# darrelllong/Delta-Compression

Measured on AMD Instinct MI355X. Metric: delta-encode GiB/s (device-resident batched pairs) at 1/2/4/8 MI355X, higher is better.
Workload: dtype u8; 1 GPU; 4096 x 64 KiB pairs per GPU, 1% edits, onepass, --table-size 1; algorithm=onepass, pairs_per_gpu=4096, pairs_total=4096, pair_bytes=65536, q=4099, parallelism=dp1 (pair shards, RCCL index scatter + size all-gather)

## Files before the change

### delta-compression_amd/__init__.py

```python
from __future__ import annotations

from ._lib import (
    ALGO_CORRECTING,
    ALGO_GREEDY,
    ALGO_ONEPASS,
    BUF_CAP,
    MAX_TABLE_SIZE,
    SEED_LEN,
    TABLE_SIZE,
    AddCmd,
    Context,
    CopyCmd,
    PlacedAdd,
    PlacedCopy,
    DeltaError,
    DiffOptions,
    EncodePlan,
    DecodePlan,
    InplacePlan,
    UpdatePlan,
    ComposeDesc,
    ComposePlan,
    InvertDesc,
    InvertPlan,
    SplicePlan,
    ReadPlan,
    ReadReq,
    ReadStream,
    SketchPlan,
    SKETCH_BINS,
    SKETCH_EMPTY,
    MATCH_NONE,
    MATCH_ALL,
    MATCH_NOT_SELF,
    MATCH_EARLIER,
    LIB_PATH,
    LIMIT_ONEPASS_MEMBERS,
    LIMIT_TABLE_POOL_BYTES,
    MEMBERS_AUTO,
    MEMBERS_OFF,
    MEMBERS_ON,
    crc64_xz,
    decode,
    decode_delta,
    default_context,
    diff,
    diff_correcting,
    diff_greedy,
    diff_onepass,
    diff_placed,
    encode,
# ... 35 lines not shown
    unplace_commands,
)

__all__ = [
    "ALGO_ONEPASS", "ALGO_CORRECTING", "ALGO_GREEDY", "SEED_LEN", "TABLE_SIZE",
    "MAX_TABLE_SIZE", "BUF_CAP", "Context", "DeltaError", "DiffOptions", "EncodePlan", "DecodePlan", "InplacePlan", "UpdatePlan",
    "ComposeDesc", "ComposePlan", "compose", "compose_batch",
    "InvertDesc", "InvertPlan", "invert", "invert_batch",
    "SplicePlan", "segment_pairs", "splice", "splice_batch", "sketch_windows", "encode_large",
    "ReadPlan", "ReadReq", "ReadStream", "read_range", "read_ranges", "tile_requests", "decode_large",
    "LineagePlan", "read_lineage", "read_lineage_batch", "lineage_work_items", "LINEAGE_BASE", "LINEAGE_MAX_DEPTH",
    "SketchPlan", "sketch", "sketch_batch", "match_sketches", "match_sketches_device", "pick_bases", "SKETCH_BINS", "SKETCH_EMPTY",
    "MATCH_NONE", "MATCH_ALL", "MATCH_NOT_SELF", "MATCH_EARLIER",
    "crc64_xz", "decode", "default_context", "encode", "encode_batch", "encode_pipelined", "info", "lib",
    "make_inplace", "make_inplace_batch", "update_batch", "status_string", "LIB_PATH", "LIMIT_TABLE_POOL_BYTES",
    "LIMIT_ONEPASS_MEMBERS", "MEMBERS_AUTO", "MEMBERS_ON", "MEMBERS_OFF",
    "CopyCmd", "AddCmd", "PlacedCopy", "PlacedAdd", "diff", "diff_greedy", "diff_onepass", "diff_correcting",
    "diff_placed", "place_commands", "unplace_commands", "output_size", "encode_delta", "decode_delta",
]
```

### delta-compression_amd/_lib.py

```python
from __future__ import annotations

import ctypes as C
import os
import threading
from dataclasses import dataclass
from typing import Iterable, List, Optional, Sequence, Tuple

HERE = os.path.dirname(os.path.abspath(__file__))
_VARIANT = os.environ.get("DG_LIB_VARIANT", "")
LIB_PATH = os.path.join(HERE, "lib", "libdeltagpu%s.so" % ("_" + _VARIANT if _VARIANT else ""))

ALGO_GREEDY, ALGO_ONEPASS, ALGO_CORRECTING = 0, 1, 2
SEED_LEN = 16
TABLE_SIZE = 1048573
MAX_TABLE_SIZE = 1073741827
BUF_CAP = 256
OPT_VERBOSE, OPT_SPLAY, OPT_INPLACE, OPT_POLICY_CONSTANT = 0, 1, 2, 3
POLICIES = {"localmin": 0, "constant": 1}
CMD_COPY, CMD_ADD = 0, 1
SKETCH_BINS = 256
SKETCH_EMPTY = 0xFFFFFFFFFFFFFFFF
MATCH_NONE = 0xFFFFFFFF
MATCH_ALL, MATCH_NOT_SELF, MATCH_EARLIER = 0, 1, 2
_MATCH_MODES = {"all": MATCH_ALL, "not_self": MATCH_NOT_SELF, "earlier": MATCH_EARLIER}

_ALGOS = {"greedy": ALGO_GREEDY, "onepass": ALGO_ONEPASS, "correcting": ALGO_CORRECTING}

STATUS = {
    0: "DG_OK", 1: "DG_ERR_INVALID_ARG", 2: "DG_ERR_UNSUPPORTED", 3: "DG_ERR_TOO_LARGE",
    4: "DG_ERR_NO_DEVICE", 5: "DG_ERR_HIP", 6: "DG_ERR_NOMEM", 7: "DG_ERR_CAPACITY",
    8: "DG_ERR_MALFORMED", 9: "DG_ERR_SRC_CRC", 10: "DG_ERR_DST_CRC", 11: "DG_ERR_TABLE_POOL", 12: "DG_ERR_INTERNAL",
}
LIMIT_TABLE_POOL_BYTES = 0
LIMIT_ONEPASS_MEMBERS = 1
MEMBERS_AUTO, MEMBERS_ON, MEMBERS_OFF = 0, 1, 2


class DeltaError(RuntimeError):
    def __init__(self, code: int, msg: str = ""):
        self.code = code
        super().__init__(f"{STATUS.get(code, code)}: {msg}" if msg else STATUS.get(code, str(code)))


class DiffOptions(C.Structure):
    _fields_ = [("p", C.c_size_t), ("q", C.c_size_t), ("buf_cap", C.c_size_t),
                ("max_table", C.c_size_t), ("flags", C.c_uint64)]

    @classmethod
    def make(cls, p: int = SEED_LEN, q: int = TABLE_SIZE, buf_cap: int = BUF_CAP,
# ... 1378 lines not shown
```

### delta-compression_amd/csrc/dg_crc.h

```cpp
#pragma once
#include <hip/hip_runtime.h>
#include <stdint.h>

#include <type_traits>

#include "dg_device.h"
#include "dg_devutil.h"

namespace dg {

typedef const __attribute__((address_space(3))) uint64_t lds_cu64;
__device__ __forceinline__ uint64_t ldsq(uint32_t a) { return *(lds_cu64*)(size_t)a; }
__device__ __forceinline__ uint32_t lds_addr(const void* p) {
	return (uint32_t)(size_t)(lds_cu64*)(const uint64_t*)p;
}

__device__ __forceinline__ uint64_t byte_mask(int lo, int hi) {
	lo = lo < 0 ? 0 : lo;
	hi = hi > 8 ? 8 : hi;
	if (hi <= lo) return 0;
	const uint64_t up = hi == 8 ? ~0ULL : ((1ULL << (8 * hi)) - 1);
	const uint64_t dn = lo == 0 ? 0ULL : ((1ULL << (8 * lo)) - 1);
	return up & ~dn;
}
// ... 55 lines not shown
		five(v, ylo, yhi, tb);
		if constexpr (PB == 16) five(v + 13, h0, h1, tb + 13 * 256);
	}
	uint32_t l[N + 1], h[N + 1];
#pragma unroll
	for (int k = 0; k < N; ++k) {
		l[k] = (uint32_t)v[k];
		h[k] = (uint32_t)(v[k] >> 32);
	}
	l[N] = xlo;
	h[N] = xhi;
	ylo = xor_tree<N + 1>(l);
	yhi = xor_tree<N + 1>(h);
}

template <uint32_t PB, uint32_t NC, int kPf, uint32_t SEG = kCrcSegBytes, bool kCopy = false, int TAB = kCrcByte>
__device__ __forceinline__ uint64_t crc_seg_rows(uintptr_t start, uint64_t len, uint32_t nseg, uint32_t j,
                                                 uint32_t tb, uint32_t tbh, uint64_t klane,
                                                 intptr_t copy_delta = 0, uintptr_t copy_hi = 0) {
	static_assert(PB == 8 || PB == 16, "piece bytes");
	static_assert(!kCopy || PB == 8, "copy: 8-byte pieces");
	static_assert(TAB == kCrcByte || NC == 1, "five-bit tables: one copy");
	constexpr uint32_t RB = 64 * PB, NR = SEG / RB;
	static_assert(NR % (2 * kPf) == 0, "two batches of rows per loop");
	const uint32_t lane = lane_id();
	const uintptr_t end = start + len;
	const uintptr_t a0 = start & ~(uintptr_t)15;
	const uintptr_t a1 = (end + 15) & ~(uintptr_t)15;
	const uintptr_t dom = a1 - (uintptr_t)nseg * SEG;
	const uintptr_t p0 = dom + (uintptr_t)j * SEG + (uintptr_t)lane * PB;
	auto clamp32 = [](intptr_t v) -> int32_t {
		return (int32_t)(v < -(intptr_t)RB ? -(intptr_t)RB : (v > (intptr_t)(SEG + RB) ? (intptr_t)(SEG + RB) : v));
	};
	const int32_t f0 = clamp32((intptr_t)start - (intptr_t)p0);
	const int32_t l0 = clamp32((intptr_t)end - (intptr_t)p0);
	const int32_t z0 = clamp32((intptr_t)a0 - (intptr_t)p0);
	typedef uint32_t v4u __attribute__((ext_vector_type(4)));
	typedef uint32_t v2u __attribute__((ext_vector_type(2)));
	typedef typename std::conditional<PB == 16, v4u, v2u>::type piece_t;
	typedef __attribute__((address_space(1))) const piece_t gpiece;
	uint32_t ylo = 0, yhi = 0, h0 = 0, h1 = 0;
	auto fold_piece = [&](const piece_t& p, uint32_t inv) {
		if constexpr (PB == 16) {
			crc_fold<TAB, PB, NC>(ylo, yhi, h0, h1, p.x ^ inv, p.y ^ inv, tb, tbh);
			h0 = p.z;
			h1 = p.w;
		} else {
			crc_fold<TAB, PB, NC>(ylo, yhi, h0, h1, p.x ^ inv, p.y ^ inv, tb, tbh);
		}
	};
	auto copy = [&](const piece_t* xs, uint32_t r0) {
		if constexpr (kCopy) {
#pragma unroll
			for (int u = 0; u < kPf; ++u) {
				const uintptr_t pa = p0 + (uintptr_t)(r0 + u) * RB;
				if (pa >= start && pa + PB <= copy_hi)
					*reinterpret_cast<__attribute__((address_space(1))) v2u*>(pa + copy_delta) = xs[u];
			}
		}
	};
	const bool edge = (j == 0 && dom != start) || (j + 1 == nseg && end != a1);
	if (!edge) {
		const uint32_t inv = j == 0 && lane == 0 ? ~0u : 0u;
		piece_t xa[kPf], xb[kPf];
		auto load = [&](piece_t* xs, uint32_t r0) {
#pragma unroll
			for (int u = 0; u < kPf; ++u) xs[u] = *reinterpret_cast<gpiece*>(p0 + (uintptr_t)(r0 + u) * RB);
		};
		auto consume = [&](const piece_t* xs, uint32_t r0) {
			copy(xs, r0);
			fold_piece(xs[0], r0 == 0 ? inv : 0u);
#pragma unroll
			for (int u = 1; u < kPf; ++u) fold_piece(xs[u], 0u);
		};
		load(xa, 0);
		for (uint32_t r0 = 0; r0 < NR; r0 += 2 * kPf) {
			load(xb, r0 + kPf);
			consume(xa, r0);
			if (r0 + 2 * kPf < NR) load(xa, r0 + 2 * kPf);
			consume(xb, r0 + kPf);
		}
	} else {
		for (uint32_t r0 = 0; r0 < NR; r0 += kPf) {
			piece_t xs[kPf];
#pragma unroll
			for (int u = 0; u < kPf; ++u) {
				const int32_t o = (int32_t)((r0 + u) * RB);
				xs[u] = piece_t{};
// ... 12 lines not shown
					const int lc = max(min(l, 24), -8);
					uint64_t lo = ((uint64_t)x.y << 32) | x.x, hi = ((uint64_t)x.w << 32) | x.z;
					lo &= byte_mask(fc, lc);
					hi &= byte_mask(fc - 8, lc - 8);
					lo ^= byte_mask(fc, fc + 8);
					hi ^= byte_mask(fc - 8, fc);
					x = v4u{(uint32_t)lo, (uint32_t)(lo >> 32), (uint32_t)hi, (uint32_t)(hi >> 32)};
				}
				piece_t px;
				if constexpr (PB == 16) px = x;
				else px = piece_t{x.x, x.y};
				fold_piece(px, 0u);
			}
		}
	}
	crc_fold<TAB, PB, NC>(ylo, yhi, h0, h1, 0u, 0u, tb, tbh);
	const uint64_t A = ((uint64_t)yhi << 32) | ylo;
	return wave_xor64(A ? gf2_mulmod(A, klane) : 0ull);
}

}
```

### delta-compression_amd/csrc/dg_device.h

```cpp
#pragma once
#include <stdint.h>

#include "../../include/delta_gpu.h"
#include "dg_layout.h"

namespace dg {


struct EncodeArgs {
	const uint8_t* ref;
	const uint8_t* ver;
	const PairDev* pairs;
	const PairPlanDev* pplan;
	uint32_t n_pairs;
	uint32_t pair0;
	uint32_t p;
	const uint64_t* powc;
	uint32_t* rec;
	uint32_t* n_rec;
	uint64_t* dsize;
	int32_t* status;
	unsigned long long* tables;
	uint64_t qmax;
	uint32_t n_tables;
// ... 90 lines not shown
	uint32_t n_pairs;
};

struct CrcArgs {
	const uint8_t* arena[2];
	const CrcSpanDev* spans;
	const CrcSegDev* segs;
	uint32_t n_segs;
	uint32_t n_spans;
	const uint64_t* tables;
	uint64_t* seg_crc;
	uint64_t* out;
	const uint64_t* xinv;
	uint64_t kseg;
	const uint32_t* prio_flag;
};

struct dg_decode_desc_dev {
	uint64_t ref_off, ref_len;
	uint64_t delta_off, delta_len;
	uint64_t out_off, out_cap;
};

struct DecodeArgs {
	const uint8_t* ref;
	const uint8_t* delta;
	const dg_decode_desc_dev* descs;
	uint32_t n;
	uint8_t* out;
	uint64_t* out_len;
// ... 17 lines not shown

hipError_t launch_onepass(const EncodeArgs& a, uint32_t p, bool aligned16, hipStream_t st,
                          hipEvent_t routed_after = nullptr);
bool onepass16_selected();
hipError_t launch_members(const SpecArgs& a, uint32_t n_chunks, uint32_t n_cu, hipStream_t st);
hipError_t launch_member_serialize(const MemSerArgs& a, uint32_t n_chunks, uint32_t n_cu, hipStream_t st);
hipError_t launch_correcting_clear(const EncodeArgs& a, hipStream_t st);
hipError_t launch_correcting(const EncodeArgs& a, uint32_t p, hipStream_t st, uint32_t lds_cap, uint64_t qmin,
                             hipEvent_t ev_built, hipEvent_t ev_fork);
hipError_t launch_greedy(const GreedyArgs& g, uint64_t head_words, hipStream_t st, hipEvent_t ev_built);
hipError_t launch_scan(const uint64_t* sz, uint64_t* off, uint32_t n, hipStream_t st,
                       uint32_t* route_cnt = nullptr, uint32_t* route_fb = nullptr);
hipError_t launch_serialize_wave(const SerArgs& s, hipStream_t st);
hipError_t launch_crc_patch(uint8_t* out, const uint64_t* offsets, const uint64_t* crc,
                            const int32_t* status, uint32_t n, hipStream_t st);
enum : int { kCrcPassRows = 0, kCrcPassRows5 = 1 };
hipError_t launch_crc(const CrcArgs& a, hipStream_t st, uint32_t overlap_cap = 0, int pass = kCrcPassRows,
                      bool finalize = true);
hipError_t launch_crc_finalize(const CrcArgs& a, hipStream_t st);
hipError_t launch_crc_wide(const CrcArgs& a, uint32_t n_cu, hipStream_t st);
hipError_t launch_decode(const DecodeArgs& a, hipStream_t st);
hipError_t launch_synth(uint8_t* ref, uint8_t* ver, uint32_t n_pairs, uint64_t pair_len,
                        uint64_t seed_base, uint64_t n_edits, hipStream_t st);
hipError_t launch_synth_shift(uint8_t* ref, uint8_t* ver, const SynthSpan* spans, const uint64_t* v_off,
                              uint32_t n, uint64_t n_edits, uint32_t pct, hipStream_t st);
hipError_t launch_synth_transpose(uint8_t* ref, uint8_t* ver, const SynthSpan* spans, uint32_t n_spans,
                                  const SynthCopy* cmds, uint32_t n_cmds, hipStream_t st);

}
```

### delta-compression_amd/csrc/dg_host.cpp

```cpp
#include <dlfcn.h>
#include <hip/hip_runtime.h>

#include <algorithm>
#include <cstdarg>
#include <cstdio>
#include <cstdlib>
#include <new>
#include <string>
#include <vector>

#include "../../include/delta_gpu.h"
#include "dg_device.h"
#include "dg_hostutil.h"
#include "dg_plan.h"

using namespace dg;


struct dg_context {
	int device = -1;
	hipStream_t stream = nullptr;
	uint64_t* d_crc_tables = nullptr;
	uint64_t* d_xinv = nullptr;
	uint64_t* d_k32 = nullptr;
	uint64_t kseg = 0;
	uint32_t n_cu = 256;
	int lds_bytes = 0;
	uint64_t table_pool_bytes = 0;
	uint64_t onepass_members = 0;
	uint64_t limits_gen = 0;
	std::string err;
	void* pin = nullptr;
	size_t pin_cap = 0;
	void* io = nullptr;
	void (*io_free)(void*) = nullptr;
	void* module[kCtxModules] = {};
	void (*module_free[kCtxModules])(void*) = {};
};

uint64_t dg::ctx_limits_gen(const dg_context_t* ctx) { return ctx->limits_gen; }
int dg::ctx_device(const dg_context_t* ctx) { return ctx->device; }

void** dg::ctx_io(dg_context_t* ctx, void (*release)(void*)) {
	ctx->io_free = release;
// ... 117 lines not shown
	delete ctx;
}

void* dg_context_stream(dg_context_t* ctx) { return ctx ? (void*)ctx->stream : nullptr; }

int dg_context_set_limit(dg_context_t* ctx, int limit, uint64_t value) {
	if (!ctx) return DG_ERR_INVALID_ARG;
	switch (limit) {
	case DG_LIMIT_TABLE_POOL_BYTES:
		ctx->table_pool_bytes = value;
		++ctx->limits_gen;
		return DG_OK;
	case DG_LIMIT_ONEPASS_MEMBERS:
		if (value > 2) return set_err(ctx, DG_ERR_INVALID_ARG, "onepass members mode %llu", (unsigned long long)value);
		ctx->onepass_members = value;
		++ctx->limits_gen;
		return DG_OK;
	default: return set_err(ctx, DG_ERR_INVALID_ARG, "unknown limit %d", limit);
	}
}

}

const char* dg::ab_env(const char* name) {
#ifdef DG_AB_SWITCHES
	return getenv(name);
#else
	(void)name;
	return nullptr;
#endif
// ... 71 lines not shown
		return 0;
	}
	uint32_t read() const { return __atomic_load_n(h, __ATOMIC_RELAXED); }
};

}


struct dg_encode_plan {
	dg_context_t* ctx = nullptr;
	dg_algorithm_t algo = DG_ALGO_ONEPASS;
	dg_diff_options_t opts{};
	uint32_t n = 0;
	EncodeGeometry g;
	std::vector<dg_pair_t> pairs;
	DevBuf d_pairs, d_pplan, d_powc, d_rec, d_nrec, d_dsize, d_crc_spans_r, d_crc_segs,
	    d_seg_crc, d_crc, d_tables, d_locks, d_tags, d_ctab, d_lookback, d_kcls, d_gpairs, d_prio_flag,
	    d_gent;
	DevBuf d_mem_s, d_srec, d_nmem, d_chunks, d_csum, d_cmap, d_seg, d_nseg;
	hipStream_t side = nullptr;
	hipEvent_t ev_fork = nullptr, ev_join = nullptr;
	bool serial_crc = false;
	bool skip_crc = false;
	DevBuf d_route_cnt;
	HostWord route_fb;
	uint32_t plain_streak = 0;
	uint64_t member_runs = 0, plain_runs = 0;
	uint64_t* stats = nullptr;
	int timing_mode = DG_TIMING_ALL;
	TimingRing ring;
// ... 15 lines not shown
#ifndef DG_CRC_PRIO_FLAG
#define DG_CRC_PRIO_FLAG 0
#endif
constexpr bool kCrcPrioFlag = DG_CRC_PRIO_FLAG != 0;

static int plan_fill(dg_encode_plan_t* P, const dg_pair_t* pairs) {
	dg_context_t* ctx = P->ctx;
	const dg_algorithm_t algo = P->algo;
	const uint32_t n = P->n;
	EncodeGeometry& g = P->g;
	PlanEnv env;
	env.n_cu = ctx->n_cu;
	env.lds_bytes = ctx->lds_bytes;
	env.table_pool_bytes = ctx->table_pool_bytes;
	env.onepass_members = ctx->onepass_members;
	env.onepass16 = onepass16_selected();
	env.no_members = ab_env("DG_NO_MEMBERS");
	env.members = ab_env("DG_MEMBERS");
	env.corr_build = ab_env("DG_CORR_BUILD");
	env.fused = ab_env("DG_FUSED");
	env.route_min = ab_env("DG_ROUTE_MIN");
	std::string err;
	const int rc = encode_geometry(algo, P->opts, pairs, n, env, g, err);
	if (rc != DG_OK) {
		if (!err.empty()) ctx->err = err;
		return rc;
	}
	hipSetDevice(ctx->device);

	const uint32_t n1 = std::max<uint32_t>(n, 1);
	const size_t p = P->opts.p;
	int bad = 0;
	bad |= P->d_pairs.alloc(sizeof(PairDev) * n1);
	bad |= P->d_pplan.alloc(sizeof(PairPlanDev) * n1);
	bad |= P->d_powc.alloc(8 * p);
	bad |= P->d_rec.alloc(4ull * (algo != DG_ALGO_CORRECTING ? kRecWordsOnepass : kRecWordsCorrecting) *
	                      std::max<uint64_t>(g.total_rec, 1));
	bad |= P->d_nrec.alloc(4ull * n1);
	bad |= P->d_dsize.alloc(8ull * n1);
	bad |= P->d_crc_spans_r.alloc(sizeof(CrcSpanDev) * std::max<size_t>(g.spans.size(), 1));
	bad |= P->d_crc_segs.alloc(sizeof(CrcSegDev) * std::max<size_t>(g.segs.size(), 1));
	bad |= P->d_seg_crc.alloc(8 * std::max<size_t>(g.segs.size(), 1));
	bad |= P->d_crc.alloc(16ull * n1);
	bad |= P->d_tables.alloc(g.table_bytes * g.n_tables);
	bad |= P->d_locks.alloc(4ull * g.n_tables);
	bad |= P->d_tags.alloc(4ull * g.n_tables);
	if (algo == DG_ALGO_CORRECTING) {
		bad |= P->d_gpairs.alloc(4ull * std::max<size_t>(g.gpairs.size(), 1));
		if (!bad && !g.gpairs.empty() &&
		    hipMemcpy(P->d_gpairs.p, g.gpairs.data(), 4 * g.gpairs.size(), hipMemcpyHostToDevice) != hipSuccess)
			bad = 1;
		bad |= P->d_ctab.alloc(4ull * std::max<uint64_t>(g.ctab_entries, 1));
		bad |= P->d_kcls.alloc(8ull * n1);
	}
	if (g.fused) bad |= P->d_lookback.alloc(8ull * n1);
	if (algo == DG_ALGO_GREEDY) {
		bad |= P->d_ctab.alloc(4ull * std::max<uint64_t>(g.greedy_heads, 1));
// ... 28 lines not shown
			g.members = false;
			g.n_chunks = 0;
			mbad = 0;
		}
		bad |= mbad;
	}
	if (bad) return set_err(ctx, DG_ERR_NOMEM, "device allocation failed");
	hipStream_t st = ctx->stream;
	hipError_t e = hipSuccess;
	if (n) {
		e = hipMemcpyAsync(P->d_pairs.p, pairs, sizeof(PairDev) * n, hipMemcpyHostToDevice, st);
		if (e == hipSuccess) e = hipMemcpyAsync(P->d_pplan.p, g.pp.data(), sizeof(PairPlanDev) * n, hipMemcpyHostToDevice, st);
		if (e == hipSuccess) e = hipMemcpyAsync(P->d_crc_spans_r.p, g.spans.data(), sizeof(CrcSpanDev) * g.spans.size(), hipMemcpyHostToDevice, st);
		if (e == hipSuccess && !g.segs.empty()) e = hipMemcpyAsync(P->d_crc_segs.p, g.segs.data(), sizeof(CrcSegDev) * g.segs.size(), hipMemcpyHostToDevice, st);
	}
	if (e == hipSuccess) e = hipMemcpyAsync(P->d_powc.p, g.powc.data(), 8 * p, hipMemcpyHostToDevice, st);
	if (e == hipSuccess) e = hipMemsetAsync(P->d_tables.p, 0, P->d_tables.n, st);
	if (e == hipSuccess) e = hipMemsetAsync(P->d_locks.p, 0, P->d_locks.n, st);
	if (e == hipSuccess) e = hipMemsetAsync(P->d_tags.p, 0, P->d_tags.n, st);
	if (e == hipSuccess) e = hipStreamSynchronize(st);
	if (e != hipSuccess) return set_err(ctx, DG_ERR_HIP, "plan upload failed: %s", hipGetErrorString(e));
	const char* sc = ab_env("DG_SERIAL_CRC");
	P->serial_crc = sc && sc[0] == '1';
	const char* sk = ab_env("DG_SKIP_CRC");
	P->skip_crc = sk && sk[0] == '1';

	if (!P->serial_crc) {
		e = hipStreamCreateWithFlags(&P->side, hipStreamNonBlocking);
		if (e == hipSuccess) e = hipEventCreateWithFlags(&P->ev_fork, hipEventDisableTiming | hipEventReleaseToDevice);
		if (e == hipSuccess) e = hipEventCreateWithFlags(&P->ev_join, hipEventDisableTiming | hipEventReleaseToDevice);
// ... 243 lines not shown
	const bool chain_join = mem && !serial && !P->skip_crc && P->g.route_min && P->route_fb.read() > 16u * ctx->n_cu;

	CrcArgs c{};
	c.arena[0] = d_ref;
	c.arena[1] = d_ver;
	c.spans = P->d_crc_spans_r.as<CrcSpanDev>();
	c.segs = P->d_crc_segs.as<CrcSegDev>();
	c.n_segs = (uint32_t)P->g.segs.size();
	c.n_spans = (uint32_t)P->g.spans.size();
	c.tables = ctx->d_crc_tables;
	c.seg_crc = P->d_seg_crc.as<uint64_t>();
	c.out = P->d_crc.as<uint64_t>();
	c.xinv = ctx->d_xinv;
	c.kseg = ctx->kseg;
	c.prio_flag = kCrcPrioFlag && mem ? P->d_prio_flag.as<uint32_t>() : nullptr;
	auto run_crc = [&]() -> int {
		HIPCHK(ctx, rec(0, cs));
		if (!P->skip_crc) {
			const uint32_t rounds = (P->n + 16u * ctx->n_cu - 1) / (16u * ctx->n_cu);
			const uint32_t cap = serial || P->g.crc_fused ? 0u : 2u * ctx->n_cu * std::max(rounds, 1u);
			HIPCHK(ctx, launch_crc(c, cs, cap, mem ? kCrcPassRows5 : kCrcPassRows, !late_fin));
		}
		HIPCHK(ctx, rec(1, cs));
		if (!serial) HIPCHK(ctx, hipEventRecord(P->ev_join, cs));
		return DG_OK;
	};
	auto run_diff = [&]() -> int {
		HIPCHK(ctx, rec(2, st));
		if (!mem) HIPCHK(ctx, rec(6, st));
		EncodeArgs a{};
		a.ref = d_ref;
		a.ver = d_ver;
		a.pairs = P->d_pairs.as<PairDev>();
		a.pplan = P->d_pplan.as<PairPlanDev>();
		a.n_pairs = P->n;
		a.p = (uint32_t)P->opts.p;
// ... 276 lines not shown
```

### delta-compression_amd/csrc/dg_kernels.hip

```cpp
#include <hip/hip_runtime.h>
#include <stdint.h>

#include <type_traits>

#include "dg_device.h"
#include "dg_devutil.h"
#include "dg_crc.h"
#include "dg_serialize_wave.h"

namespace dg {


__device__ __forceinline__ uint64_t wave_incl_scan64(uint64_t x) {
	const uint32_t lane = lane_id();
#pragma unroll
	for (int d = 1; d < 64; d <<= 1) {
		const uint32_t lo = (uint32_t)__shfl_up((int)(uint32_t)x, d, 64);
		const uint32_t hi = (uint32_t)__shfl_up((int)(uint32_t)(x >> 32), d, 64);
		if (lane >= (uint32_t)d) x += ((uint64_t)hi << 32) | lo;
	}
	return x;
}

__global__ __launch_bounds__(1024) void scan_sizes_kernel(const uint64_t* __restrict__ sz,
// ... 73 lines not shown
	for (uint32_t seg = uni(blockIdx.x * kCrcWavesPerBlock + wave); seg < a.n_segs;
	     seg += gridDim.x * kCrcWavesPerBlock) {
		if (a.prio_flag && !raised) {
			if (uni(__hip_atomic_load(a.prio_flag, __ATOMIC_RELAXED, __HIP_MEMORY_SCOPE_AGENT))) {
				__builtin_amdgcn_s_setprio(1);
				raised = true;
			}
		}
		const CrcSegDev sd = a.segs[seg];
		const CrcSpanDev sp = a.spans[sd.span];
		const uint64_t c = crc_seg_rows<8, 1, TAB == kCrcByte ? DG_CRC_PF : DG_CRC_PF5, kCrcSegBytes, false, TAB>(
		    (uintptr_t)(a.arena[sp.which] + sp.off), sp.len, sp.nseg, sd.j, tb, tb, kl);
		if (lane == 0) a.seg_crc[seg] = c;
	}
}

__global__ __launch_bounds__(64) void crc_finalize_kernel(CrcArgs a) {
	const uint32_t i = blockIdx.x * 64 + threadIdx.x;
	if (i >= a.n_spans) return;
	const CrcSpanDev sp = a.spans[i];
	uint64_t crc;
	if (sp.len < 8) {
		const uint8_t* d = a.arena[sp.which] + sp.off;
		uint64_t c = ~0ULL;
		for (uint64_t k = 0; k < sp.len; ++k) c = a.tables[(uint8_t)(c ^ d[k])] ^ (c >> 8);
		crc = ~c;
	} else {
		const uint64_t* KS = a.tables + 8 * 256 + kCrcLevels * kCrcNibTabWords;
		uint64_t acc = 0;
		for (uint32_t j = 0; j < sp.nseg; ++j)
// ... 223 lines not shown

hipError_t launch_crc_finalize(const CrcArgs& a, hipStream_t st) {
	if (a.n_spans) hipLaunchKernelGGL(crc_finalize_kernel, dim3((a.n_spans + 63) / 64), dim3(64), 0, st, a);
	return hipGetLastError();
}

hipError_t launch_crc(const CrcArgs& a, hipStream_t st, uint32_t overlap_cap, int pass, bool finalize) {
	if (a.n_segs) {
		uint32_t blocks = (a.n_segs + kCrcWavesPerBlock - 1) / kCrcWavesPerBlock;
		static const uint32_t env_cap = [] {
			const char* e = ab_env("DG_CRC_BLOCKS");
			return e ? (uint32_t)strtoul(e, nullptr, 0) : 0u;
		}();
		const uint32_t cap = env_cap ? env_cap : overlap_cap;
		if (cap && blocks > cap) blocks = cap;
		if (pass == kCrcPassRows5)
			hipLaunchKernelGGL(crc_rows_kernel<kCrcFive>, dim3(blocks), dim3(64 * kCrcWavesPerBlock), 0, st, a);
		else
			hipLaunchKernelGGL(crc_rows_kernel<kCrcByte>, dim3(blocks), dim3(64 * kCrcWavesPerBlock), 0, st, a);
	}
	if (finalize) return launch_crc_finalize(a, st);
	return hipGetLastError();
}

hipError_t launch_synth(uint8_t* ref, uint8_t* ver, uint32_t n_pairs, uint64_t pair_len,
                        uint64_t seed_base, uint64_t n_edits, hipStream_t st) {
	const uint64_t words = (uint64_t)n_pairs * ((pair_len + 7) / 8);
	if (words)
		hipLaunchKernelGGL(synth_random_kernel, dim3((unsigned)((words + 255) / 256)), dim3(256), 0, st,
		                   ref, ver, pair_len, seed_base, words);
// ... 233 lines not shown
```

### delta-compression_amd/csrc/dg_layout.h

```cpp
#pragma once
#include <stdint.h>

namespace dg {

constexpr uint64_t kMersenne = (1ULL << 61) - 1;
constexpr uint64_t kBase = 263;
constexpr uint64_t kCrcPoly = 0xC96C5795D7870F42ULL;
constexpr uint32_t kSentinel = 0xFFFFFFFFu;

constexpr uint32_t kCrcSegBytes = 65536;
constexpr uint32_t kCrcWavesPerBlock = 4;

#ifndef DG_HIST_CHUNKS
#define DG_HIST_CHUNKS 6
#endif
constexpr int kHistChunks = DG_HIST_CHUNKS;

struct PairDev {
	uint64_t r_off, r_len, v_off, v_len;
};

struct PairPlanDev {
	uint64_t q;
	uint64_t q_magic;
// ... 2 lines not shown
	uint32_t pad;
	uint64_t f_size, f_magic;
	uint64_t m, m_magic;
	uint64_t tab_base;
	uint64_t mem_base;
	uint32_t chunk_base;
	uint32_t n_chunks;
	uint64_t crc_unpad;
};

struct CrcSegDev {
	uint32_t span;
	uint32_t j;
};

struct CrcSpanDev {
	uint64_t off, len;
	uint32_t seg_base;
	uint32_t nseg;
	uint32_t which;
	uint32_t out;
};

constexpr int kCrcLevels = 6;
constexpr int kCrcNibTabWords = 256;
constexpr int kCrcFinTabs = 1 + 16 + 3 + 3;
constexpr int kCrcFinX256 = 20, kCrcFinX512 = 21, kCrcFinX48K = 22;
constexpr uint32_t kCrcRowsOff = 8 * 256 + (kCrcLevels + kCrcFinTabs) * kCrcNibTabWords;
constexpr uint32_t kCrcRows16 = kCrcRowsOff, kCrcRows8 = kCrcRowsOff + 16 * 256;
constexpr uint32_t kCrcRowK16 = kCrcRowsOff + 24 * 256, kCrcRowK8 = kCrcRowK16 + 64;
// ... 22 lines not shown
```

### delta-compression_amd/csrc/dg_plan.cpp

```cpp
#include "dg_plan.h"

#include <algorithm>
#include <cstdarg>
#include <cstdio>
#include <cstdlib>
#include <cstring>
#include <map>

namespace dg {


namespace {

typedef unsigned __int128 u128;

uint64_t mulmod64(uint64_t a, uint64_t b, uint64_t m) { return (uint64_t)((u128)a * b % m); }

uint64_t powmod64(uint64_t b, uint64_t e, uint64_t m) {
	uint64_t r = 1 % m;
	b %= m;
	for (; e; e >>= 1) {
		if (e & 1) r = mulmod64(r, b, m);
		b = mulmod64(b, b, m);
	}
// ... 157 lines not shown
	seg.clear();
	for (size_t i = 0; i < spans.size(); ++i) {
		CrcSpanDev& s = sd[i];
		s.off = spans[i].off;
		s.len = spans[i].len;
		s.seg_base = (uint32_t)seg.size();
		s.nseg = 0;
		s.which = which[i];
		s.out = outs ? (*outs)[i] : (uint32_t)i;
		if (s.len >= 8) {
			const uint64_t a0 = s.off & ~15ull, a1 = (s.off + s.len + 15) & ~15ull;
			s.nseg = (uint32_t)((a1 - a0 + kCrcSegBytes - 1) / kCrcSegBytes);
			for (uint32_t j = 0; j < s.nseg; ++j) seg.push_back(CrcSegDev{(uint32_t)i, j});
		}
	}
}


namespace {

bool is_one(const char* v) { return v && v[0] == '1'; }

bool members_wanted(const PlanEnv& env, const dg_pair_t* pairs, uint32_t n) {
	uint64_t vsum = 0;
	for (uint32_t i = 0; i < n; ++i) vsum += pairs[i].v_len;
	bool want = n && vsum / n >= (128u << 10);
	if (env.onepass_members == 1) want = true;
	if (env.onepass_members == 2) want = false;
	if (is_one(env.no_members)) want = false;
	if (is_one(env.members)) want = true;
// ... 147 lines not shown
	if (g.members) {
		for (uint32_t i = 0; i < n; ++i) {
			const uint64_t E = std::min<uint64_t>(pairs[i].r_len, pairs[i].v_len);
			const uint32_t nch = (uint32_t)(E / kMemChunk + 1);
			g.pp[i].mem_base = g.mem_slots;
			g.pp[i].chunk_base = g.n_chunks;
			g.pp[i].n_chunks = nch;
			for (uint32_t c = 0; c < nch; ++c) {
				g.jobs.push_back(i);
				g.jobs.push_back(c);
			}
			g.mem_slots += (uint64_t)nch * kMemChunkSlots;
			g.n_chunks += nch;
		}
	}
	return DG_OK;
}


namespace {
void print_command_stats(const dg_commands_t& cmds) {
	uint64_t tc = 0, ta = 0, nc = 0, na = 0;
	std::vector<uint64_t> lens;
	for (size_t i = 0; i < cmds.len; ++i) {
		const dg_placed_command_t& c = cmds.data[i];
		if (c.tag == DG_CMD_COPY) { tc += c.length; ++nc; lens.push_back(c.length); }
		else { ta += c.length; ++na; }
	}
	const uint64_t tot = tc + ta;
	fprintf(stderr,
// ... 313 lines not shown
```

### delta-compression_amd/csrc/dg_plan.h

```cpp
#pragma once
#include <stdint.h>

#include <string>
#include <vector>

#include "../../include/delta_gpu.h"
#include "dg_compose_dev.h"
#include "dg_inplace_dev.h"
#include "dg_invert_dev.h"
#include "dg_layout.h"
#include "dg_sketch_dev.h"
#include "dg_splice_dev.h"

namespace dg {

bool is_prime_u64(uint64_t n);
uint64_t next_prime(uint64_t n);
uint64_t gf2_mul(uint64_t a, uint64_t b);
uint64_t gf2_pow(uint64_t base, uint64_t e);
uint64_t gf2_xpow(uint64_t n);
uint64_t gf2_div_x(uint64_t z);

struct CrcTables {
	std::vector<uint64_t> tab;
	uint64_t xinv[16];
	uint64_t k32[1024];
	uint64_t kseg;
};
void crc_tables_build(CrcTables& t);

void plan_crc_spans(const std::vector<dg_span_t>& spans, const std::vector<uint32_t>& which,
                    std::vector<CrcSpanDev>& sd, std::vector<CrcSegDev>& seg,
                    const std::vector<uint32_t>* outs = nullptr);

struct PlanEnv {
	uint32_t n_cu = 256;
	int lds_bytes = 0;
	uint64_t table_pool_bytes = 0;
	uint64_t onepass_members = 0;
	bool onepass16 = true;
	const char* no_members = nullptr;
	const char* members = nullptr;
	const char* corr_build = nullptr;
	const char* fused = nullptr;
	const char* route_min = nullptr;
};

struct EncodeGeometry {
	std::vector<PairPlanDev> pp;
	uint64_t out_bound = 0;
	uint64_t total_rec = 0;
	uint64_t qmax = 0, qmin = ~0ull;
	uint64_t ctab_entries = 0;
	uint64_t greedy_heads = 0;
	uint64_t greedy_entries = 0;
	uint64_t max_seeds = 0;
	bool aligned16 = true;
	uint64_t v_total = 0;
	std::vector<uint64_t> powc;
	uint32_t corr_lds_cap = 0;
	bool crc_fused = false;
	std::vector<uint32_t> gpairs;
	std::vector<CrcSpanDev> spans;
	std::vector<CrcSegDev> segs;
	uint64_t table_bytes = 0;
	uint32_t n_tables = 0;
	bool fused = false;
	bool members = false;
	uint32_t route_min = 0;
	std::vector<uint32_t> jobs;
	uint64_t mem_slots = 0;
	uint32_t n_chunks = 0;
};

int encode_geometry(dg_algorithm_t algo, const dg_diff_options_t& o, const dg_pair_t* pairs, uint32_t n,
                    const PlanEnv& env, EncodeGeometry& g, std::string& err);

uint64_t pair_out_bound(dg_algorithm_t algo, uint64_t p, uint64_t v_len);

// ... 58 lines not shown
```

### include/delta_gpu.h

```cpp
#ifndef DELTA_GPU_H
#define DELTA_GPU_H

#include <stddef.h>
#include <stdint.h>

#ifdef __cplusplus
extern "C" {
#endif

#define DG_ABI_VERSION 3

#define DG_SEED_LEN        16
#define DG_TABLE_SIZE      1048573UL
#define DG_MAX_TABLE_SIZE  1073741827UL
#define DG_BUF_CAP         256
#define DG_HEADER_SIZE     25
#define DG_CRC_SIZE        8

typedef enum {
	DG_OK              = 0,
	DG_ERR_INVALID_ARG = 1,
	DG_ERR_UNSUPPORTED = 2,
	DG_ERR_TOO_LARGE   = 3,
	DG_ERR_NO_DEVICE   = 4,
// ... 35 lines not shown

void dg_buffer_free(dg_buffer_t *buf);


typedef struct dg_context dg_context_t;

int  dg_context_create(int device, dg_context_t **out);
void dg_context_destroy(dg_context_t *ctx);
void *dg_context_stream(dg_context_t *ctx);
const char *dg_status_string(int status);
const char *dg_last_error(const dg_context_t *ctx);
int dg_abi_version(void);

#define DG_LIMIT_TABLE_POOL_BYTES 0
#define DG_LIMIT_ONEPASS_MEMBERS 1
int dg_context_set_limit(dg_context_t *ctx, int limit, uint64_t value);

typedef struct {
	uint64_t r_off;
	uint64_t r_len;
	uint64_t v_off;
	uint64_t v_len;
} dg_pair_t;

typedef struct dg_encode_plan dg_encode_plan_t;

int dg_encode_plan_create(dg_context_t *ctx, dg_algorithm_t algo,
                          const dg_pair_t *pairs , uint32_t n_pairs,
                          const dg_diff_options_t *opts,
                          dg_encode_plan_t **out);
// ... 415 lines not shown
```

Before: 1889 GiB/s.

## Add wave-walk CRC kernel interleaving several segments per wave

Adds a CRC pass in which each wave walks up to four same-index segments from different spans in round-robin slices, carrying a separate fold state for each. A host planner groups the segments and assigns them to waves. The goal is to hide memory latency by keeping several independent load streams in flight per wave, and to balance work across waves. It also adds a CRC block-count limit/env knob and moves the cap calculation into the planner. The walk path is compiled only when DG_CRC_WALK is defined, and it adds register pressure and planning cost.

```diff
diff --git a/delta-compression_amd/__init__.py b/delta-compression_amd/__init__.py
--- a/delta-compression_amd/__init__.py
+++ b/delta-compression_amd/__init__.py
@@ -35,6 +35,7 @@
     MATCH_NOT_SELF,
     MATCH_EARLIER,
     LIB_PATH,
+    LIMIT_CRC_BLOCKS,
     LIMIT_ONEPASS_MEMBERS,
     LIMIT_TABLE_POOL_BYTES,
     MEMBERS_AUTO,
@@ -100,7 +101,7 @@
     "MATCH_NONE", "MATCH_ALL", "MATCH_NOT_SELF", "MATCH_EARLIER",
     "crc64_xz", "decode", "default_context", "encode", "encode_batch", "encode_pipelined", "info", "lib",
     "make_inplace", "make_inplace_batch", "update_batch", "status_string", "LIB_PATH", "LIMIT_TABLE_POOL_BYTES",
-    "LIMIT_ONEPASS_MEMBERS", "MEMBERS_AUTO", "MEMBERS_ON", "MEMBERS_OFF",
+    "LIMIT_ONEPASS_MEMBERS", "LIMIT_CRC_BLOCKS", "MEMBERS_AUTO", "MEMBERS_ON", "MEMBERS_OFF",
     "CopyCmd", "AddCmd", "PlacedCopy", "PlacedAdd", "diff", "diff_greedy", "diff_onepass", "diff_correcting",
     "diff_placed", "place_commands", "unplace_commands", "output_size", "encode_delta", "decode_delta",
 ]
diff --git a/delta-compression_amd/_lib.py b/delta-compression_amd/_lib.py
--- a/delta-compression_amd/_lib.py
+++ b/delta-compression_amd/_lib.py
@@ -33,6 +33,7 @@
 }
 LIMIT_TABLE_POOL_BYTES = 0
 LIMIT_ONEPASS_MEMBERS = 1
+LIMIT_CRC_BLOCKS = 2
 MEMBERS_AUTO, MEMBERS_ON, MEMBERS_OFF = 0, 1, 2
 
 
diff --git a/delta-compression_amd/csrc/dg_crc.h b/delta-compression_amd/csrc/dg_crc.h
--- a/delta-compression_amd/csrc/dg_crc.h
+++ b/delta-compression_amd/csrc/dg_crc.h
@@ -93,14 +93,49 @@
 	yhi = xor_tree<N + 1>(h);
 }
 
+template <uint32_t PB, uint32_t NC, int kPf, int TAB>
+struct CrcRowFold {
+	static_assert(PB == 8 || PB == 16, "piece bytes");
+	static_assert(TAB == kCrcByte || NC == 1, "five-bit tables: one copy");
+	static constexpr uint32_t RB = 64 * PB;
+	typedef uint32_t v4u __attribute__((ext_vector_type(4)));
+	typedef uint32_t v2u __attribute__((ext_vector_type(2)));
+	typedef typename std::conditional<PB == 16, v4u, v2u>::type piece_t;
+	typedef __attribute__((address_space(1))) const piece_t gpiece;
+	uint32_t ylo = 0, yhi = 0, h0 = 0, h1 = 0;
+
+	__device__ __forceinline__ void fold_piece(const piece_t& p, uint32_t inv, uint32_t tb, uint32_t tbh) {
+		if constexpr (PB == 16) {
+			crc_fold<TAB, PB, NC>(ylo, yhi, h0, h1, p.x ^ inv, p.y ^ inv, tb, tbh);
+			h0 = p.z;
+			h1 = p.w;
+		} else {
+			crc_fold<TAB, PB, NC>(ylo, yhi, h0, h1, p.x ^ inv, p.y ^ inv, tb, tbh);
+		}
+	}
+	static __device__ __forceinline__ void load(piece_t* xs, uintptr_t p) {
+#pragma unroll
+		for (int u = 0; u < kPf; ++u) xs[u] = *reinterpret_cast<gpiece*>(p + (uintptr_t)u * RB);
+	}
+	__device__ __forceinline__ void consume(const piece_t* xs, uint32_t inv, uint32_t tb, uint32_t tbh) {
+		fold_piece(xs[0], inv, tb, tbh);
+#pragma unroll
+		for (int u = 1; u < kPf; ++u) fold_piece(xs[u], 0u, tb, tbh);
+	}
+	__device__ __forceinline__ uint64_t finish(uint32_t tb, uint32_t tbh, uint64_t klane) {
+		crc_fold<TAB, PB, NC>(ylo, yhi, h0, h1, 0u, 0u, tb, tbh);
+		const uint64_t A = ((uint64_t)yhi << 32) | ylo;
+		return wave_xor64(A ? gf2_mulmod(A, klane) : 0ull);
+	}
+};
+
 template <uint32_t PB, uint32_t NC, int kPf, uint32_t SEG = kCrcSegBytes, bool kCopy = false, int TAB = kCrcByte>
 __device__ __forceinline__ uint64_t crc_seg_rows(uintptr_t start, uint64_t len, uint32_t nseg, uint32_t j,
                                                  uint32_t tb, uint32_t tbh, uint64_t klane,
                                                  intptr_t copy_delta = 0, uintptr_t copy_hi = 0) {
-	static_assert(PB == 8 || PB == 16, "piece bytes");
 	static_assert(!kCopy || PB == 8, "copy: 8-byte pieces");
-	static_assert(TAB == kCrcByte || NC == 1, "five-bit tables: one copy");
-	constexpr uint32_t RB = 64 * PB, NR = SEG / RB;
+	typedef CrcRowFold<PB, NC, kPf, TAB> Fold;
+	constexpr uint32_t RB = Fold::RB, NR = SEG / RB;
 	static_assert(NR % (2 * kPf) == 0, "two batches of rows per loop");
 	const uint32_t lane = lane_id();
 	const uintptr_t end = start + len;
@@ -114,20 +149,12 @@
 	const int32_t f0 = clamp32((intptr_t)start - (intptr_t)p0);
 	const int32_t l0 = clamp32((intptr_t)end - (intptr_t)p0);
 	const int32_t z0 = clamp32((intptr_t)a0 - (intptr_t)p0);
-	typedef uint32_t v4u __attribute__((ext_vector_type(4)));
-	typedef uint32_t v2u __attribute__((ext_vector_type(2)));
-	typedef typename std::conditional<PB == 16, v4u, v2u>::type piece_t;
-	typedef __attribute__((address_space(1))) const piece_t gpiece;
-	uint32_t ylo = 0, yhi = 0, h0 = 0, h1 = 0;
-	auto fold_piece = [&](const piece_t& p, uint32_t inv) {
-		if constexpr (PB == 16) {
-			crc_fold<TAB, PB, NC>(ylo, yhi, h0, h1, p.x ^ inv, p.y ^ inv, tb, tbh);
-			h0 = p.z;
-			h1 = p.w;
-		} else {
-			crc_fold<TAB, PB, NC>(ylo, yhi, h0, h1, p.x ^ inv, p.y ^ inv, tb, tbh);
-		}
-	};
+	typedef typename Fold::v4u v4u;
+	typedef typename Fold::v2u v2u;
+	typedef typename Fold::piece_t piece_t;
+	typedef typename Fold::gpiece gpiece;
+	Fold f;
+	auto fold_piece = [&](const piece_t& p, uint32_t inv) { f.fold_piece(p, inv, tb, tbh); };
 	auto copy = [&](const piece_t* xs, uint32_t r0) {
 		if constexpr (kCopy) {
 #pragma unroll
@@ -138,19 +165,15 @@
 			}
 		}
 	};
-	const bool edge = (j == 0 && dom != start) || (j + 1 == nseg && end != a1);
+	const bool edge = (j == 0 && dom != start) || (j + 1 == nseg && end != a1) ||
+	                  (j == 1 && (uintptr_t)SEG - (start - dom) < 8);
 	if (!edge) {
 		const uint32_t inv = j == 0 && lane == 0 ? ~0u : 0u;
 		piece_t xa[kPf], xb[kPf];
-		auto load = [&](piece_t* xs, uint32_t r0) {
-#pragma unroll
-			for (int u = 0; u < kPf; ++u) xs[u] = *reinterpret_cast<gpiece*>(p0 + (uintptr_t)(r0 + u) * RB);
-		};
+		auto load = [&](piece_t* xs, uint32_t r0) { Fold::load(xs, p0 + (uintptr_t)r0 * RB); };
 		auto consume = [&](const piece_t* xs, uint32_t r0) {
 			copy(xs, r0);
-			fold_piece(xs[0], r0 == 0 ? inv : 0u);
-#pragma unroll
-			for (int u = 1; u < kPf; ++u) fold_piece(xs[u], 0u);
+			f.consume(xs, r0 == 0 ? inv : 0u, tb, tbh);
 		};
 		load(xa, 0);
 		for (uint32_t r0 = 0; r0 < NR; r0 += 2 * kPf) {
@@ -193,9 +216,7 @@
 			}
 		}
 	}
-	crc_fold<TAB, PB, NC>(ylo, yhi, h0, h1, 0u, 0u, tb, tbh);
-	const uint64_t A = ((uint64_t)yhi << 32) | ylo;
-	return wave_xor64(A ? gf2_mulmod(A, klane) : 0ull);
-}
-
-}
+	return f.finish(tb, tbh, klane);
+}
+
+}
diff --git a/delta-compression_amd/csrc/dg_device.h b/delta-compression_amd/csrc/dg_device.h
--- a/delta-compression_amd/csrc/dg_device.h
+++ b/delta-compression_amd/csrc/dg_device.h
@@ -128,6 +128,9 @@
 	const uint64_t* xinv;
 	uint64_t kseg;
 	const uint32_t* prio_flag;
+	const CrcWalkDev* walk;
+	const uint32_t* walk_first;
+	uint32_t n_walk_waves;
 };
 
 struct dg_decode_desc_dev {
@@ -175,7 +178,7 @@
 hipError_t launch_serialize_wave(const SerArgs& s, hipStream_t st);
 hipError_t launch_crc_patch(uint8_t* out, const uint64_t* offsets, const uint64_t* crc,
                             const int32_t* status, uint32_t n, hipStream_t st);
-enum : int { kCrcPassRows = 0, kCrcPassRows5 = 1 };
+enum : int { kCrcPassRows = 0, kCrcPassRows5 = 1, kCrcPassWalk = 2 };
 hipError_t launch_crc(const CrcArgs& a, hipStream_t st, uint32_t overlap_cap = 0, int pass = kCrcPassRows,
                       bool finalize = true);
 hipError_t launch_crc_finalize(const CrcArgs& a, hipStream_t st);
diff --git a/delta-compression_amd/csrc/dg_host.cpp b/delta-compression_amd/csrc/dg_host.cpp
--- a/delta-compression_amd/csrc/dg_host.cpp
+++ b/delta-compression_amd/csrc/dg_host.cpp
@@ -28,6 +28,7 @@
 	int lds_bytes = 0;
 	uint64_t table_pool_bytes = 0;
 	uint64_t onepass_members = 0;
+	uint64_t crc_blocks = 0;
 	uint64_t limits_gen = 0;
 	std::string err;
 	void* pin = nullptr;
@@ -175,6 +176,10 @@
 	case DG_LIMIT_ONEPASS_MEMBERS:
 		if (value > 2) return set_err(ctx, DG_ERR_INVALID_ARG, "onepass members mode %llu", (unsigned long long)value);
 		ctx->onepass_members = value;
+		++ctx->limits_gen;
+		return DG_OK;
+	case DG_LIMIT_CRC_BLOCKS:
+		ctx->crc_blocks = value;
 		++ctx->limits_gen;
 		return DG_OK;
 	default: return set_err(ctx, DG_ERR_INVALID_ARG, "unknown limit %d", limit);
@@ -276,6 +281,7 @@
 	uint32_t n = 0;
 	EncodeGeometry g;
 	std::vector<dg_pair_t> pairs;
+	DevBuf d_crc_walk, d_crc_walk_first;
 	DevBuf d_pairs, d_pplan, d_powc, d_rec, d_nrec, d_dsize, d_crc_spans_r, d_crc_segs,
 	    d_seg_crc, d_crc, d_tables, d_locks, d_tags, d_ctab, d_lookback, d_kcls, d_gpairs, d_prio_flag,
 	    d_gent;
@@ -321,6 +327,9 @@
 	env.lds_bytes = ctx->lds_bytes;
 	env.table_pool_bytes = ctx->table_pool_bytes;
 	env.onepass_members = ctx->onepass_members;
+	env.crc_blocks = ctx->crc_blocks;
+	if (!env.crc_blocks)
+		if (const char* e = ab_env("DG_CRC_BLOCKS")) env.crc_blocks = strtoull(e, nullptr, 0);
 	env.onepass16 = onepass16_selected();
 	env.no_members = ab_env("DG_NO_MEMBERS");
 	env.members = ab_env("DG_MEMBERS");
@@ -348,6 +357,10 @@
 	bad |= P->d_crc_spans_r.alloc(sizeof(CrcSpanDev) * std::max<size_t>(g.spans.size(), 1));
 	bad |= P->d_crc_segs.alloc(sizeof(CrcSegDev) * std::max<size_t>(g.segs.size(), 1));
 	bad |= P->d_seg_crc.alloc(8 * std::max<size_t>(g.segs.size(), 1));
+	if (g.walk_waves) {
+		bad |= P->d_crc_walk.alloc(sizeof(CrcWalkDev) * std::max<size_t>(g.walk.size(), 1));
+		bad |= P->d_crc_walk_first.alloc(4 * g.walk_first.size());
+	}
 	bad |= P->d_crc.alloc(16ull * n1);
 	bad |= P->d_tables.alloc(g.table_bytes * g.n_tables);
 	bad |= P->d_locks.alloc(4ull * g.n_tables);
@@ -406,6 +419,10 @@
 		if (e == hipSuccess) e = hipMemcpyAsync(P->d_crc_spans_r.p, g.spans.data(), sizeof(CrcSpanDev) * g.spans.size(), hipMemcpyHostToDevice, st);
 		if (e == hipSuccess && !g.segs.empty()) e = hipMemcpyAsync(P->d_crc_segs.p, g.segs.data(), sizeof(CrcSegDev) * g.segs.size(), hipMemcpyHostToDevice, st);
 	}
+	if (e == hipSuccess && g.walk_waves) {
+		if (!g.walk.empty()) e = hipMemcpyAsync(P->d_crc_walk.p, g.walk.data(), sizeof(CrcWalkDev) * g.walk.size(), hipMemcpyHostToDevice, st);
+		if (e == hipSuccess) e = hipMemcpyAsync(P->d_crc_walk_first.p, g.walk_first.data(), 4 * g.walk_first.size(), hipMemcpyHostToDevice, st);
+	}
 	if (e == hipSuccess) e = hipMemcpyAsync(P->d_powc.p, g.powc.data(), 8 * p, hipMemcpyHostToDevice, st);
 	if (e == hipSuccess) e = hipMemsetAsync(P->d_tables.p, 0, P->d_tables.n, st);
 	if (e == hipSuccess) e = hipMemsetAsync(P->d_locks.p, 0, P->d_locks.n, st);
@@ -679,12 +696,21 @@
 	c.xinv = ctx->d_xinv;
 	c.kseg = ctx->kseg;
 	c.prio_flag = kCrcPrioFlag && mem ? P->d_prio_flag.as<uint32_t>() : nullptr;
+	static const bool walk_off = [] {
+		const char* e = ab_env("DG_CRC_WALK");
+		return e && e[0] == '0';
+	}();
+	const bool walk = P->g.walk_waves && !mem && !serial && !walk_off;
+	if (walk) {
+		c.walk = P->d_crc_walk.as<CrcWalkDev>();
+		c.walk_first = P->d_crc_walk_first.as<uint32_t>();
+		c.n_walk_waves = P->g.walk_waves;
+	}
 	auto run_crc = [&]() -> int {
 		HIPCHK(ctx, rec(0, cs));
 		if (!P->skip_crc) {
-			const uint32_t rounds = (P->n + 16u * ctx->n_cu - 1) / (16u * ctx->n_cu);
-			const uint32_t cap = serial || P->g.crc_fused ? 0u : 2u * ctx->n_cu * std::max(rounds, 1u);
-			HIPCHK(ctx, launch_crc(c, cs, cap, mem ? kCrcPassRows5 : kCrcPassRows, !late_fin));
+			const uint32_t cap = serial ? 0u : P->g.crc_cap;
+			HIPCHK(ctx, launch_crc(c, cs, cap, walk ? kCrcPassWalk : mem ? kCrcPassRows5 : kCrcPassRows, !late_fin));
 		}
 		HIPCHK(ctx, rec(1, cs));
 		if (!serial) HIPCHK(ctx, hipEventRecord(P->ev_join, cs));
diff --git a/delta-compression_amd/csrc/dg_kernels.hip b/delta-compression_amd/csrc/dg_kernels.hip
--- a/delta-compression_amd/csrc/dg_kernels.hip
+++ b/delta-compression_amd/csrc/dg_kernels.hip
@@ -111,6 +111,101 @@
 		if (lane == 0) a.seg_crc[seg] = c;
 	}
 }
+
+#ifdef DG_CRC_WALK
+template <int N, int kPf, int TAB>
+__device__ __forceinline__ void crc_walk_group(const CrcArgs& a, const CrcWalkDev& wd, uint32_t tb, uint64_t kl) {
+	typedef CrcRowFold<8, 1, kPf, TAB> Fold;
+	typedef typename Fold::piece_t piece_t;
+	constexpr uint32_t RB = Fold::RB, NR = kCrcSegBytes / RB, SL = 2 * kPf * DG_CRC_WALK_SLICE;
+	static_assert(NR % SL == 0 && (SL & (SL - 1)) == 0, "whole slices");
+	const uint32_t lane = lane_id();
+	__amdgpu_buffer_rsrc_t seg[N];
+	Fold f[N];
+	uint32_t inv = 0;
+#pragma unroll
+	for (int k = 0; k < N; ++k) {
+		const CrcSegDev sd = a.segs[wd.seg[k]];
+		const CrcSpanDev sp = a.spans[sd.span];
+		const uintptr_t end = (uintptr_t)(a.arena[sp.which] + sp.off) + sp.len;
+		const uintptr_t a1 = (end + 15) & ~(uintptr_t)15;
+		const uintptr_t base = uni64(a1 - (uintptr_t)(sp.nseg - sd.j) * kCrcSegBytes);
+		seg[k] = __builtin_amdgcn_make_buffer_rsrc((void*)base, (short)0, (int)kCrcSegBytes, 0x00020000);
+		if (sd.j == 0 && lane == 0) inv = ~0u;
+	}
+	const int lo = (int)(lane * 8u);
+	auto load = [&](piece_t* xs, const __amdgpu_buffer_rsrc_t& r, uint32_t row) {
+#pragma unroll
+		for (int u = 0; u < kPf; ++u)
+			xs[u] = __builtin_bit_cast(piece_t, __builtin_amdgcn_raw_buffer_load_b64(r, lo + u * (int)RB, (int)(row * RB), 0));
+	};
+	piece_t xa[kPf], xb[kPf];
+	load(xa, seg[0], 0);
+	uint32_t k = 0;
+#pragma nounroll
+	for (uint32_t r = 0; r < NR;) {
+		load(xb, seg[0], r + kPf);
+		f[0].consume(xa, r == 0 ? inv : 0u, tb, tb);
+		const bool turn_ends = (r + 2 * kPf) % SL == 0;
+		const uint32_t rn = !turn_ends || k + 1 == N ? r + 2 * kPf : r + 2 * kPf - SL;
+		if (rn < NR) load(xa, turn_ends ? seg[N > 1 ? 1 : 0] : seg[0], rn);
+		f[0].consume(xb, 0u, tb, tb);
+		if (turn_ends) {
+			const Fold f0 = f[0];
+			const __amdgpu_buffer_rsrc_t s0 = seg[0];
+#pragma unroll
+			for (int i = 0; i + 1 < N; ++i) {
+				f[i] = f[i + 1];
+				seg[i] = seg[i + 1];
+			}
+			f[N - 1] = f0;
+			seg[N - 1] = s0;
+			k = k + 1 < N ? k + 1 : 0;
+		}
+		r = rn;
+	}
+#pragma unroll
+	for (int k = 0; k < N; ++k) {
+		const uint64_t c = f[k].finish(tb, tb, kl);
+		if (lane == 0) a.seg_crc[wd.seg[k]] = c;
+	}
+}
+
+template <int TAB>
+__global__ __launch_bounds__(256, DG_CRC_MINBLOCKS) void crc_rows_walk_kernel(CrcArgs a) {
+	if constexpr (DG_CRC_PRIO > 0) __builtin_amdgcn_s_setprio(DG_CRC_PRIO);
+	constexpr uint32_t nt = TAB == kCrcByte ? 8 * 256 : 32 * kCrc5Tabs8;
+	constexpr int kPf = TAB == kCrcByte ? DG_CRC_PF : DG_CRC_PF5;
+	__shared__ __attribute__((aligned(256))) uint64_t T8[nt];
+	for (uint32_t i = threadIdx.x; i < nt; i += 256) T8[i] = a.tables[(TAB == kCrcByte ? kCrcRows8 : kCrc5R8) + i];
+	__syncthreads();
+	const uint32_t wave = threadIdx.x >> 6, lane = lane_id();
+	const uint32_t tb = lds_addr(T8);
+	const uint64_t kl = a.tables[kCrcRowK8 + lane];
+	for (uint32_t wv = uni(blockIdx.x * kCrcWavesPerBlock + wave); wv < a.n_walk_waves;
+	     wv += gridDim.x * kCrcWavesPerBlock) {
+		const uint32_t g1 = uni(a.walk_first[wv + 1]);
+		for (uint32_t g = uni(a.walk_first[wv]); g < g1; ++g) {
+			const CrcWalkDev wd = a.walk[g];
+			const uint32_t n = uni(wd.n);
+			if (uni(wd.edge) || n == 1) {
+				const CrcSegDev sd = a.segs[wd.seg[0]];
+				const CrcSpanDev sp = a.spans[sd.span];
+				const uint64_t c = crc_seg_rows<8, 1, kPf, kCrcSegBytes, false, TAB>(
+				    (uintptr_t)(a.arena[sp.which] + sp.off), sp.len, sp.nseg, sd.j, tb, tb, kl);
+				if (lane == 0) a.seg_crc[wd.seg[0]] = c;
+			} else if (n == 2) {
+				crc_walk_group<2, kPf, TAB>(a, wd, tb, kl);
+			} else if (n == 3) {
+				crc_walk_group<3, kPf, TAB>(a, wd, tb, kl);
+			} else if (n == 4) {
+				crc_walk_group<4, kPf, TAB>(a, wd, tb, kl);
+			}
+		}
+	}
+}
+static_assert(kCrcWalkG == 4, "crc_rows_walk_kernel dispatches groups of up to 4");
+#endif
 
 __global__ __launch_bounds__(64) void crc_finalize_kernel(CrcArgs a) {
 	const uint32_t i = blockIdx.x * 64 + threadIdx.x;
@@ -364,6 +459,11 @@
 		}();
 		const uint32_t cap = env_cap ? env_cap : overlap_cap;
 		if (cap && blocks > cap) blocks = cap;
+#ifdef DG_CRC_WALK
+		if (pass == kCrcPassWalk)
+			hipLaunchKernelGGL(crc_rows_walk_kernel<kCrcByte>, dim3(blocks), dim3(64 * kCrcWavesPerBlock), 0, st, a);
+		else
+#endif
 		if (pass == kCrcPassRows5)
 			hipLaunchKernelGGL(crc_rows_kernel<kCrcFive>, dim3(blocks), dim3(64 * kCrcWavesPerBlock), 0, st, a);
 		else
diff --git a/delta-compression_amd/csrc/dg_layout.h b/delta-compression_amd/csrc/dg_layout.h
--- a/delta-compression_amd/csrc/dg_layout.h
+++ b/delta-compression_amd/csrc/dg_layout.h
@@ -40,6 +40,21 @@
 	uint32_t j;
 };
 
+constexpr uint32_t kCrcWalkG = 4;
+#ifndef DG_CRC_WALK_FILL
+#define DG_CRC_WALK_FILL 4
+#endif
+#ifndef DG_CRC_WALK_SLICE
+#define DG_CRC_WALK_SLICE 1
+#endif
+constexpr uint32_t kCrcWalkFill = DG_CRC_WALK_FILL;
+static_assert(kCrcWalkFill >= 1 && kCrcWalkFill <= kCrcWalkG, "group fill");
+struct CrcWalkDev {
+	uint32_t seg[kCrcWalkG];
+	uint32_t n;
+	uint32_t edge;
+};
+
 struct CrcSpanDev {
 	uint64_t off, len;
 	uint32_t seg_base;
diff --git a/delta-compression_amd/csrc/dg_plan.cpp b/delta-compression_amd/csrc/dg_plan.cpp
--- a/delta-compression_amd/csrc/dg_plan.cpp
+++ b/delta-compression_amd/csrc/dg_plan.cpp
@@ -195,6 +195,64 @@
 			for (uint32_t j = 0; j < s.nseg; ++j) seg.push_back(CrcSegDev{(uint32_t)i, j});
 		}
 	}
+}
+
+void plan_crc_walk(const std::vector<CrcSpanDev>& sd, const std::vector<CrcSegDev>& seg, uint32_t n_waves,
+                   std::vector<CrcWalkDev>& groups, std::vector<uint32_t>& first) {
+	(void)seg;
+	n_waves = std::max(n_waves, 1u);
+	struct Run {
+		uint32_t span, j0, n;
+	};
+	std::vector<Run> runs;
+	std::vector<uint32_t> edges;
+	for (size_t i = 0; i < sd.size(); ++i) {
+		const CrcSpanDev& s = sd[i];
+		if (!s.nseg) continue;
+		const uint64_t end = s.off + s.len, a1 = (end + 15) & ~15ull;
+		const uint64_t dom = a1 - (uint64_t)s.nseg * kCrcSegBytes;
+		uint32_t j0 = 0, j1 = s.nseg;
+		if (dom != s.off) {
+			edges.push_back(s.seg_base + j0++);
+			if (j1 > j0 && kCrcSegBytes - (s.off - dom) < 8) edges.push_back(s.seg_base + j0++);
+		}
+		if (end != a1 && j1 > j0) edges.push_back(s.seg_base + --j1);
+		if (j1 > j0) runs.push_back(Run{(uint32_t)i, j0, j1 - j0});
+	}
+	std::stable_sort(runs.begin(), runs.end(),
+	                 [](const Run& a, const Run& b) { return a.j0 != b.j0 ? a.j0 < b.j0 : a.n < b.n; });
+	const uint32_t g = (uint32_t)std::min<uint64_t>(kCrcWalkFill, std::max<uint64_t>(1, (runs.size() + n_waves - 1) / n_waves));
+	std::vector<std::vector<CrcWalkDev>> per(n_waves);
+	uint32_t w = 0;
+	for (size_t b = 0; b < runs.size();) {
+		size_t e = b + 1;
+		while (e < runs.size() && e - b < g && runs[e].j0 == runs[b].j0) ++e;
+		uint32_t steps = 0;
+		for (size_t k = b; k < e; ++k) steps = std::max(steps, runs[k].n);
+		for (uint32_t t = 0; t < steps; ++t) {
+			CrcWalkDev d{};
+			for (size_t k = b; k < e; ++k)
+				if (t < runs[k].n) d.seg[d.n++] = sd[runs[k].span].seg_base + runs[k].j0 + t;
+			per[w].push_back(d);
+		}
+		w = (w + 1) % n_waves;
+		b = e;
+	}
+	for (uint32_t s : edges) {
+		CrcWalkDev d{};
+		d.seg[0] = s;
+		d.n = 1;
+		d.edge = 1;
+		per[w].push_back(d);
+		w = (w + 1) % n_waves;
+	}
+	groups.clear();
+	first.assign(n_waves + 1, 0);
+	for (uint32_t k = 0; k < n_waves; ++k) {
+		first[k] = (uint32_t)groups.size();
+		groups.insert(groups.end(), per[k].begin(), per[k].end());
+	}
+	first[n_waves] = (uint32_t)groups.size();
 }
 
 
@@ -372,6 +430,19 @@
 			g.n_chunks += nch;
 		}
 	}
+	{
+		const uint32_t rounds = (n + 16u * env.n_cu - 1) / (16u * env.n_cu);
+		g.crc_cap = g.crc_fused ? 0u : 2u * env.n_cu * std::max(rounds, 1u);
+		if (env.crc_blocks) g.crc_cap = (uint32_t)std::min<uint64_t>(env.crc_blocks, 0x7fffffffu);
+#ifdef DG_CRC_WALK
+		if (algo == DG_ALGO_ONEPASS && !g.members && !g.segs.empty()) {
+			uint32_t blocks = (uint32_t)((g.segs.size() + kCrcWavesPerBlock - 1) / kCrcWavesPerBlock);
+			if (g.crc_cap) blocks = std::min(blocks, g.crc_cap);
+			g.walk_waves = blocks * kCrcWavesPerBlock;
+			plan_crc_walk(g.spans, g.segs, g.walk_waves, g.walk, g.walk_first);
+		}
+#endif
+	}
 	return DG_OK;
 }
 
diff --git a/delta-compression_amd/csrc/dg_plan.h b/delta-compression_amd/csrc/dg_plan.h
--- a/delta-compression_amd/csrc/dg_plan.h
+++ b/delta-compression_amd/csrc/dg_plan.h
@@ -33,11 +33,15 @@
                     std::vector<CrcSpanDev>& sd, std::vector<CrcSegDev>& seg,
                     const std::vector<uint32_t>* outs = nullptr);
 
+void plan_crc_walk(const std::vector<CrcSpanDev>& sd, const std::vector<CrcSegDev>& seg, uint32_t n_waves,
+                   std::vector<CrcWalkDev>& groups, std::vector<uint32_t>& first);
+
 struct PlanEnv {
 	uint32_t n_cu = 256;
 	int lds_bytes = 0;
 	uint64_t table_pool_bytes = 0;
 	uint64_t onepass_members = 0;
+	uint64_t crc_blocks = 0;
 	bool onepass16 = true;
 	const char* no_members = nullptr;
 	const char* members = nullptr;
@@ -63,6 +67,10 @@
 	std::vector<uint32_t> gpairs;
 	std::vector<CrcSpanDev> spans;
 	std::vector<CrcSegDev> segs;
+	uint32_t crc_cap = 0;
+	uint32_t walk_waves = 0;
+	std::vector<CrcWalkDev> walk;
+	std::vector<uint32_t> walk_first;
 	uint64_t table_bytes = 0;
 	uint32_t n_tables = 0;
 	bool fused = false;
diff --git a/include/delta_gpu.h b/include/delta_gpu.h
--- a/include/delta_gpu.h
+++ b/include/delta_gpu.h
@@ -73,6 +73,7 @@
 
 #define DG_LIMIT_TABLE_POOL_BYTES 0
 #define DG_LIMIT_ONEPASS_MEMBERS 1
+#define DG_LIMIT_CRC_BLOCKS 2
 int dg_context_set_limit(dg_context_t *ctx, int limit, uint64_t value);
 
 typedef struct {
```

Result: slower. 1862 GiB/s (-1.4%).
